# pmorenoz/HetMOGP

Measured on AMD Instinct MI355X. Metric: ELBO-steps/sec (one step = ELBO + all parameter gradients), higher is better.
Workload: dtype f64

## Files before the change

### hetmogp_amd/csrc/common.h

```cpp
#pragma once
#include <hip/hip_runtime.h>
#include <stdint.h>
#include <string>

#define HMOGP_WAVE 64
#ifndef HMOGP_POTRF_NB
#define HMOGP_POTRF_NB 32
#endif

typedef double f64x4 __attribute__((ext_vector_type(4)));
typedef double f64x2 __attribute__((ext_vector_type(2)));

struct HipError {
  hipError_t code;
  const char* what;
  const char* file;
  int line;
};
#define HIP_TRY(expr)                                          \
  do {                                                         \
    hipError_t _e = (expr);                                    \
    if (_e != hipSuccess) throw HipError{_e, #expr, __FILE__, __LINE__}; \
  } while (0)

// ... 7 lines not shown
  v = wave_sum(v);
  const int lane = threadIdx.x & 63, w = threadIdx.x >> 6, nw = (blockDim.x + 63) >> 6;
  __syncthreads();
  if (lane == 0) scratch[w] = v;
  __syncthreads();
  double r = 0.0;
  if (threadIdx.x == 0)
    for (int i = 0; i < nw; ++i) r += scratch[i];
  return r;
}

struct GemmArgs {
  const double* A = nullptr;
  const double* B = nullptr;
  double* C = nullptr;
  const double* kscale = nullptr;
  int M = 0, N = 0, K = 0;
  int lda = 0, ldb = 0, ldc = 0;
  long long sA = 0, sB = 0, sC = 0, sS = 0;
  double alpha = 1.0, beta = 0.0;
  int nbatch = 1;
  int M_last = 0, N_last = 0, K_last = 0;
  int nouter = 1;
  long long oA = 0, oB = 0, oC = 0, oS = 0;
  int ksplit = 1;
  long long sSplit = 0;
  int a_kmajor = 0, b_kmajor = 1;
  int lower_only = 0;
  int diag_balance = 1;
  int role = 0;
  double* fs_part = nullptr;
  const double* fs_a = nullptr;
  const double* fs_x = nullptr;
  const double* fs_z = nullptr;
  const double* fs_ell = nullptr;
  int fs_ldz = 0, fs_P = 1, fs_hyper = 0;
  long long fs_sPart = 0, fs_sA = 0, fs_sZ = 0;
  int store_c = 1;
  int fs_sq = 0;
  const double* fs_k = nullptr;
  const double* c_src = nullptr;
  int c_sub = 0;
  int a_tri = 0, b_tri = 0;
  const int* win = nullptr;
  long long win_stride = 0;
};
void launch_combine_parts(const double* part, int tiles, long long n, double* p, double* c, double* pt, double* ct,
                          hipStream_t s, int nb = 1, long long sPart = 0, long long ldn = 0);
void launch_gemm_f64(const GemmArgs& g, hipStream_t stream);
bool gemm_rowpass_eligible(const GemmArgs& g);
void launch_gemm_rowpass(const GemmArgs& g, hipStream_t stream);
int launch_gemm_rowpass_or_general(const GemmArgs& g, hipStream_t stream);
bool gemm_rowpass_would_take(const GemmArgs& g);
constexpr int GEMM_MAX_FWD_PARTS = 4;
bool gemm_small_eligible(const GemmArgs& g);
void launch_gemm_small(const GemmArgs& g, hipStream_t stream);

void launch_potrf_batched(double* A, int Q, int M, int* d_info, double* dscr, hipStream_t stream, int panel_begin = 0,
                          int panel_end = -1);
void launch_trtri_batched(const double* L, double* Linv, double* tmp, int Q, int M, hipStream_t stream, bool linv_is_zero = false);
void launch_ltl_batched(const double* Linv, double* Out, int Q, int M, hipStream_t stream);

void launch_fill(double* p, long long n, double v, hipStream_t stream);
void launch_unpack_tril(const double* L_flat , double* L , int Q, int M, hipStream_t s);
void launch_gemv_batched(const double* A, const double* x, double* y, int Q, int M, long long sx, int incx,
                         hipStream_t s);
```

### hetmogp_amd/csrc/engine.hip

```cpp
#include "engine_impl.h"

hipEvent_t hmogp_engine::new_event() {
  if (pool_used == pool.size()) {
    hipEvent_t e;
    HIP_TRY(hipEventCreate(&e));
    pool.push_back(e);
  }
  return pool[pool_used++];
}

void hmogp_engine::collect_spans() {
  static const bool dbg = getenv("HMOGP_DEBUG_TIMELINE") != nullptr;
  for (auto& s : spans) {
    float f = 0.f;
    if (hipEventElapsedTime(&f, s.a, s.b) == hipSuccess) ms[s.cat] += f;
    if (dbg) {
      float t0 = 0.f;
      if (hipEventElapsedTime(&t0, ev_begin0, s.a) == hipSuccess)
        std::fprintf(stderr, "[hmogp timeline] cat %d  start %9.3f ms  dur %9.3f ms\n", s.cat, t0, f);
    }
  }
  spans.clear();
  pool_used = 0;
}

hmogp_engine::~hmogp_engine() {
  drop_graphs();
  comm_destroy();
  for (auto e : pool) (void)hipEventDestroy(e);
  if (h_info2) (void)hipHostFree(h_info2);
  if (ev_ng) (void)hipEventDestroy(ev_ng);
  if (h_small) (void)hipHostFree(h_small);
  for (auto e : {ev_begin0, ev_begin1, ev_fin0, ev_fin1, ev_fork, ev_gsk, ev_zero, ev_info, ev_S, ev_join, ev_col, ev_kuf, ev_params, ev_ua, ev_qu})
    if (e) (void)hipEventDestroy(e);
  if (hstage) (void)hipHostFree(hstage);
  if (h_info) (void)hipHostFree(h_info);
  if (h_cond) (void)hipHostFree(h_cond);
  if (ev_cond) (void)hipEventDestroy(ev_cond);
  if (st2_own) (void)hipStreamDestroy(st2_own);
  if (st3_own) (void)hipStreamDestroy(st3_own);
  if (st) (void)hipStreamDestroy(st);
}

void hmogp_engine::init(const hmogp_config* c) {
  if (!c || c->abi_version != HMOGP_ABI_VERSION) throw EngineError{HMOGP_E_INVALID, "bad config / ABI version"};
  T = c->T, Q = c->Q, M = c->M, P = c->P, Df = c->Df, device = c->device;
  if (T < 1 || Q < 1 || M < 1 || Df < 1) throw EngineError{HMOGP_E_INVALID, "T, Q, M, Df must be >= 1"};
  if (P < 1 || P > 4) throw EngineError{HMOGP_E_INVALID, "input dimension P must be 1..4"};
  if (Q > HMOGP_MAXQ) throw EngineError{HMOGP_E_INVALID, "Q exceeds HMOGP_MAXQ (8)"};
  if (c->chunk_rows > 0) {
    chunk = c->chunk_rows;
  } else {
    const long long fit = (64LL << 30) / (16LL * Q * M);
    chunk = std::max<long long>(4096, std::min<long long>(1048576, fit / 1024 * 1024));
  }
  use_windows = (c->flags & HMOGP_CFG_EXACT_ZERO_WINDOWS) != 0;
  cache_kuu = (c->flags & HMOGP_CFG_CACHE_KUU) != 0;
  no_small = (c->flags & HMOGP_CFG_NO_SMALL_PATH) != 0;
  strict = strict_cfg = (c->flags & HMOGP_CFG_STRICT_QF) != 0;
  if (strict && use_windows) throw EngineError{HMOGP_E_INVALID, "HMOGP_CFG_STRICT_QF and HMOGP_CFG_EXACT_ZERO_WINDOWS exclude each other"};
  if (c->flags & ~(HMOGP_CFG_EXACT_ZERO_WINDOWS | HMOGP_CFG_CACHE_KUU | HMOGP_CFG_NO_SMALL_PATH | HMOGP_CFG_STRICT_QF))
    throw EngineError{HMOGP_E_INVALID, "unknown bits in hmogp_config.flags"};
  quirks = c->quirks;
  if (quirks & ~HMOGP_QUIRKS_REFERENCE) throw EngineError{HMOGP_E_INVALID, "unknown bits in hmogp_config.quirks"};
  if (use_windows && M > 8192) throw EngineError{HMOGP_E_INVALID, "exact-zero windows support M <= 8192"};
  int ndev = 0;
  if (hipGetDeviceCount(&ndev) != hipSuccess || ndev < 1)
    throw EngineError{HMOGP_E_NO_DEVICE, "no HIP device visible (this library has no CPU path)"};
  if (device < 0 || device >= ndev) throw EngineError{HMOGP_E_NO_DEVICE, "HIP device ordinal out of range"};
  HIP_TRY(hipSetDevice(device));
  {
    int lo = 0, hi = 0;
    HIP_TRY(hipDeviceGetStreamPriorityRange(&lo, &hi));
    HIP_TRY(hipStreamCreateWithPriority(&st, hipStreamNonBlocking, hi));
    const char* cus_env = getenv("HMOGP_ST2_CUS");
    int cus = cus_env ? atoi(cus_env) : 0;
    hipDeviceProp_t prop;
    HIP_TRY(hipGetDeviceProperties(&prop, device));
    if (cus > 0 && cus < prop.multiProcessorCount) {
      std::vector<uint32_t> mask((prop.multiProcessorCount + 31) / 32, 0u);
      for (int i = 0; i < cus; ++i) mask[i / 32] |= 1u << (i % 32);
      if (hipExtStreamCreateWithCUMask(&st2, (uint32_t)mask.size(), mask.data()) != hipSuccess) st2 = nullptr;
    }
    const char* free_env = getenv("HMOGP_ST2_FREE");
    const int nfree = free_env ? atoi(free_env) : 0;
    if (!st2 && nfree > 0 && nfree < 32 && prop.multiProcessorCount == 256) {
      const char* lay = getenv("HMOGP_ST2_LAYOUT");
      const int layout = lay ? atoi(lay) : 1;
      st2_masked = true;
      std::vector<uint32_t> mask(8, 0xFFFFFFFFu);
      for (int x = 0; x < 8; ++x)
        for (int c = 32 - nfree; c < 32; ++c) {
          const int bit = layout == 0 ? x * 32 + c : c * 8 + x;
          mask[bit / 32] &= ~(1u << (bit % 32));
        }
      if (hipExtStreamCreateWithCUMask(&st2, (uint32_t)mask.size(), mask.data()) != hipSuccess) st2 = nullptr, st2_masked = false;
    }
    if (!st2) HIP_TRY(hipStreamCreateWithPriority(&st2, hipStreamNonBlocking, lo));
    HIP_TRY(hipStreamCreateWithPriority(&st3, hipStreamNonBlocking, hi));
    st2_own = st2, st3_own = st3;
  }
  for (hipEvent_t* e : {&ev_fork, &ev_gsk, &ev_zero, &ev_info, &ev_S, &ev_join, &ev_col, &ev_kuf, &ev_params, &ev_ua, &ev_qu})
    HIP_TRY(hipEventCreateWithFlags(e, hipEventDisableTiming));
  HIP_TRY(hipEventRecord(ev_qu, st));
  HIP_TRY(hipEventRecord(ev_join, st));
  for (hipEvent_t* e : {&ev_begin0, &ev_begin1, &ev_fin0, &ev_fin1}) HIP_TRY(hipEventCreate(e));
  f_index.assign(c->f_index, c->f_index + Df);
  d_index.assign(c->d_index, c->d_index + Df);
  tasks.resize(T);
  int d = 0;
  for (int t = 0; t < T; ++t) {
    Task& k = tasks[t];
    k.lik = c->lik_id[t];
    k.param = c->lik_param ? c->lik_param[t] : 0.0;
    if (k.lik == HMOGP_LIK_GAUSSIAN && !(k.param > 0.0)) k.param = 0.5;
    k.dimf = lik_dimf(k.lik, k.param);
    check_lik_param(k.lik, k.param);
    k.qparam = k.lik == HMOGP_LIK_ORDINAL ? ordinal_table(k.param).sigma : k.param;
    if (k.dimf < 1 || k.dimf > HMOGP_MAXJ) throw EngineError{HMOGP_E_INVALID, "unsupported likelihood / dim_f"};
    k.d0 = d;
    for (int j = 0; j < k.dimf; ++j, ++d)
      if (d >= Df || f_index[d] != t || d_index[d] != j)
        throw EngineError{HMOGP_E_INVALID, "f_index / d_index inconsistent with the likelihood list"};
  }
  if (d != Df) throw EngineError{HMOGP_E_INVALID, "Df does not match the likelihood list"};
  const long long MM = (long long)M * M;
  NG = 2 + Df;
  oR = MM, oDZ = MM + M, oSA = oDZ + (long long)M * P, oSL = oSA + 1, oSWK = oSA + 2;
  per_q = oSWK + Df;
  nstats = NG + Q * per_q;
  stats.ensure(sizeof(double) * nstats, true);
  nwire = NG + Q * ((long long)M * (M + 1) / 2 + (per_q - MM));
  for (int t = 0; t < T; ++t) {
    Task& k = tasks[t];
    const int J = k.dimf;
    k.nscal = 2 + 2 * Q + J + Q * J;
    std::vector<long long> off(k.nscal);
    off[0] = 0, off[1] = 1;
    for (int q = 0; q < Q; ++q) {
      off[2 + 2 * q] = NG + q * per_q + oSA;
      off[3 + 2 * q] = NG + q * per_q + oSL;
      for (int j = 0; j < J; ++j) off[2 + 2 * Q + J + q * J + j] = NG + q * per_q + oSWK + k.d0 + j;
    }
    for (int j = 0; j < J; ++j) off[2 + 2 * Q + j] = 2 + k.d0 + j;
    k.offsets.ensure(sizeof(long long) * k.nscal);
    HIP_TRY(hipMemcpy(k.offsets.p, off.data(), sizeof(long long) * k.nscal, hipMemcpyHostToDevice));
  }
  const size_t mmq = sizeof(double) * MM * Q;
  for (DevBuf* b : {&Kuu, &Luu, &Kuui, &L, &S, &KiS, &KSK, &C, &Ctri, &Sqi, &tmpA, &tmpB, &HK, &G, &GSK, &dKmm, &dLdS}) b->ensure(mmq, true);
  oJit = 2 * Q + 2 * Q * Df, oW0 = oJit + Q, oBs = oW0 + Q * Df, oSeq = oBs + T;
  n_small = oSeq + 1;
  auto even = [](long long n) { return (n + 1) & ~1LL; };
  const long long nZ = (long long)M * Q * P, nmu = (long long)M * Q, nL = ((long long)M * (M + 1) / 2) * Q;
  oZ = even(n_small), oMu = oZ + even(nZ), oLf = oMu + even(nmu), n_params = oLf + even(nL);
  dparams.ensure(sizeof(double) * n_params);
// ... 456 lines not shown
```

### hetmogp_amd/csrc/engine_impl.h

```cpp
#pragma once
#include <algorithm>
#include <cmath>
#include <cstdio>
#include <cstdlib>
#include <cstring>
#include <string>
#include <vector>

#include <chrono>
#include <thread>

#include <dlfcn.h>
#include <hip/hip_runtime.h>
extern "C" {
typedef struct ncclComm* ncclComm_t;
}
namespace hm_nccl {
struct UniqueId { char internal[128]; };
enum : int { Success = 0, InProgress = 7, DataDouble = 8, OpSum = 0 };
using GetUniqueId = int (*)(UniqueId*);
using CommInitRank = int (*)(ncclComm_t*, int, UniqueId, int);
using CommDestroy = int (*)(ncclComm_t);
using CommAbort = int (*)(ncclComm_t);
using CommGetAsyncError = int (*)(ncclComm_t, int*);
// ... 170 lines not shown
  long long n_small = 0, oZ = 0, oMu = 0, oLf = 0, n_params = 0, oJit = 0, oW0 = 0, oBs = 0, oSeq = 0;
  int eval_seq = 0;
  DevBuf Kuu, Luu, Kuui, L, S, KiS, KSK, C, Ctri, Sqi, tmpA, tmpB, HK, G, GSK, dKmm, dLdS;
  DevBuf a, Kr, gmu, gL, klout, rowout, dinfo, djit, dscr;
  long long ws_rows = 0;
  DevBuf Kh, Pt, vp, vc, vpt, vct, valpha, vbeta, valpha0, vbeta0;
  DevBuf colred;
  DevBuf stats, wire, slabs, colpart, quadpart, fwdpart, winrow, wincol, winhit, Xws, dstage;
  long long nwire = 0;
  int* h_info = nullptr;
  double* hstage = nullptr;
  size_t hstage_cap = 0;
  bool began = false, evaluated = false;
  bool qu_resident = false;
  DevBuf ad_gms_m, ad_sms_m, ad_step_m, ad_pend_m, ad_gms_L, ad_sms_L, ad_step_L, ad_pend_L;

  struct Span {
    hipEvent_t a, b;
    int cat;
  };
  std::vector<hipEvent_t> pool;
  size_t pool_used = 0;
  std::vector<Span> spans;
  double ms[NCAT] = {0};
  long long launches[NCAT] = {0};
  hipEvent_t ev_begin0 = nullptr, ev_begin1 = nullptr, ev_fin0 = nullptr, ev_fin1 = nullptr;
  bool st2_masked = false;
  hipStream_t st2_own = nullptr, st3_own = nullptr;
  bool small_mode = false;
  bool small_path = false, small_veto = false, small_info_pending = false, info_early = false;
  double* hstage_dev = nullptr;
  bool small_rows = false;
  DevBuf smallslab;
  struct RetryRegular {};
  struct SmallGraph {
    std::vector<long long> key;
    hipGraph_t graph = nullptr;
    hipGraphExec_t exec = nullptr;
  };
  std::vector<SmallGraph> graphs;
  std::vector<std::vector<long long>> warm_keys;
  long long graph_replays = 0, graph_captures = 0;
  void drop_graphs(bool keep_warm = false);
  std::vector<long long> graph_key(const hmogp_params* p) const;
  bool graph_step(const hmogp_params* p, hmogp_outputs* out);
  bool graphs_broken = false, via_graph = false;
  std::vector<long long> pending_warm;
  void mark_warm();
  hipStream_t st2 = nullptr;
  hipStream_t st3 = nullptr;
  hipEvent_t ev_qu = nullptr;
  hipEvent_t ev_fork = nullptr, ev_gsk = nullptr, ev_zero = nullptr, ev_info = nullptr, ev_S = nullptr, ev_join = nullptr, ev_col = nullptr, ev_kuf = nullptr, ev_params = nullptr,
             ev_ua = nullptr;

  hipEvent_t new_event();
  struct Scope {
    hmogp_engine* e;
    Span s;
    hipStream_t stream;
    bool on_;
    Scope(hmogp_engine* eng, int cat, int nlaunch, hipStream_t on = nullptr) : e(eng), stream(on ? on : eng->st) {
      static const bool off = getenv("HMOGP_NO_SPANS") != nullptr;
      on_ = !off && (!eng->small_mode || cat == CAT_EXCHANGE);
      s.cat = cat;
      e->launches[cat] += nlaunch;
      if (!on_) return;
      s.a = e->new_event();
      s.b = e->new_event();
      (void)hipEventRecord(s.a, stream);
    }
    ~Scope() {
      if (!on_) return;
      (void)hipEventRecord(s.b, stream);
      e->spans.push_back(s);
    }
  };
  void collect_spans();

  ncclComm_t comm = nullptr;
  int comm_ranks = 1, comm_rank = 0;
  bool exchanged = false;

  void comm_init(int nranks, int rank, const void* id);
  void comm_destroy();
  void comm_abort();
  void wait_exchanged();
  void exchange();

  ~hmogp_engine();

  double* Hq(int q) { return stats.d() + NG + q * per_q; }

  void init(const hmogp_config* c);

  void set_task_data(int t, const double* X, const double* Y, long long N);

  void ensure_workspace(long long rows);

  long long ws_strict_rows = 0;
  void ensure_strict_workspace();

  void upload_params(const hmogp_params* p, bool enqueue = true);

  void mm(const double* A, bool a_k, const double* B, bool b_k, double* Cc, double alpha = 1.0, long long sA = -1,
          int lda = -1, hipStream_t stream = nullptr, int a_tri = 0, int b_tri = 0, bool lower_only = false) {
    GemmArgs g;
// ... 72 lines not shown
```

### hetmogp_amd/csrc/engine_rows.hip

```cpp
#include "engine_impl.h"

void hmogp_engine::u_algebra_small() {
  Scope sc(this, CAT_MM, 1);
  kuu_key_valid = false;
  if (!h_info) HIP_TRY(hipHostMalloc((void**)&h_info, sizeof(int) * HMOGP_MAXQ, hipHostMallocDefault));
  for (int q = 0; q < Q; ++q)
    if (rung[q] == -2) rung[q] = -1;
  if (!pools.empty()) {
    stage_pool_inputs(pools[0], st);
    if (!small_rows) kuf_pool(pools[0], st);
    kuf_prefetched = true;
    HIP_TRY(hipEventRecord(ev_kuf, st));
  }
  SmallU u;
  u.M = M, u.Q = Q, u.P = P, u.ldz = Q * P;
  u.Z = dZ.d(), u.var = dvar.d(), u.ell = dell.d(), u.jit = dsmall.d() + oJit, u.mu = dmu.d(), u.Lflat = dLflat.d();
  u.Kuu = Kuu.d(), u.Luu = Luu.d(), u.Kuui = Kuui.d(), u.L = L.d(), u.S = S.d(), u.KiS = KiS.d(), u.KSK = KSK.d(), u.C = C.d();
  u.Ctri = Ctri.d(), u.Sqi = Sqi.d(), u.a = a.d(), u.klout = klout.d(), u.info = dinfo.as<int>(), u.flag = dinfo.as<int>() + HMOGP_MAXQ;
  u.seq = dsmall.d() + oSeq;
  u.zero = stats.d(), u.nzero = nstats;
  launch_u_small(u, st);
  if (info_early) HIP_TRY(hipMemcpyAsync(h_info, dinfo.p, sizeof(int) * Q, hipMemcpyDeviceToHost, st));
  small_info_pending = true;
  HIP_TRY(hipEventRecord(ev_join, st));
// ... 424 lines not shown
      const bool row_sl = want_hyper && !col_sl;
      qm.p = vp.d(), qm.c = vc.d(), qm.pt = row_sl ? vpt.d() : nullptr, qm.ct = row_sl ? vct.d() : nullptr;
      qm.Wd = dW.d(), qm.W0d = dsmall.d() + oW0, qm.kapd = dkap.d(), qm.vard = dvar.d(), qm.scale_base = dsmall.d() + oBs;
      qm.quirks = quirks;
      qm.alpha = valpha.d(), qm.beta = vbeta.d(), qm.alpha0 = valpha0.d(), qm.beta0 = vbeta0.d(), qm.partials = quadpart.d();
      long long part = 0;
      for (size_t i = 0; i < pl.size(); ++i) {
        const Seg& sg = pl[i];
        Task& k = tasks[sg.t];
        QuadSeg& g = qm.seg[i];
        g.lik = k.lik, g.dimf = k.dimf, g.d0 = k.d0, g.t = sg.t, g.lik_param = k.qparam, g.N = sg.n, g.off = sg.off;
        g.y = k.quad_y() + sg.r0, g.yaux = k.Yaux.p ? k.Yaux.d() + sg.r0 : nullptr, g.ldy = k.quad_ldy();
        auto& r = qred.s[qred.nseg++];
        r.part = quadpart.d() + part, r.nrows = quad_blocks(k.lik, sg.n), r.nscal = k.nscal, r.off = k.offsets.as<long long>();
        part += r.nrows * k.nscal;
      }
      if (quad_multi || quad_multi_specialised(qm)) {
        Scope sc(this, CAT_QUAD, quad_multi ? 1 : 2);
        launch_quad_multi(qm, st);
        if (!quad_multi) launch_reduce_rows_multi(qred, stats.d(), st);
      } else {
        Scope sc(this, CAT_QUAD, 2 * (int)pl.size());
        for (auto& sg : pl) quad_segment(sg);
      }
    } else {
      Scope sc(this, CAT_QUAD, 2 * (int)pl.size());
      for (auto& sg : pl) quad_segment(sg);
    }
    if (small_rows) {
      Scope sc(this, CAT_GRAM, 2);
      launch_small_bwd(sr, st, quad_multi ? &qred : nullptr);
      continue;
    }
    colstats_rows(0, n, 0);
    {
      const int ksplit = use_windows ? std::min(8, gram_ksplit(n, M)) : gram_ksplit(n, M);
      slabs.ensure(sizeof(double) * MM * ksplit * Q, true);
      GemmArgs g;
      g.A = strict ? Ah.d() : Kh.d(), g.lda = M, g.a_kmajor = 1, g.sA = sK;
      g.B = g.A, g.ldb = M, g.b_kmajor = 1, g.sB = sK;
      g.kscale = vbeta.d(), g.sS = ldn;
      g.C = slabs.d(), g.ldc = M, g.sC = MM * ksplit;
      g.M = g.N = M, g.K = (int)n;
      g.nbatch = Q;
      g.lower_only = 1;
      g.ksplit = ksplit, g.sSplit = MM;
      g.role = 2;
      static const int bal = [] {
        const char* e = getenv("HMOGP_DIAG_BALANCE");
        return e ? atoi(e) : 1;
      }();
      g.diag_balance = bal;
      g.win = cw, g.win_stride = 2 * ncb;
      {
        Scope sc(this, CAT_GRAM, 1);
        launch_gemm_rowpass_or_general(g, st);
      }
      {
        Scope sc(this, CAT_COLSTATS, 1, st2);
        launch_reduce_slabs(colpart.d(), (int)nsp, clen, (long long)M * (1 + P), Hq(0) + oR, true, st2, Q, nsp * clen, per_q);
        if (col_sl) {
          launch_reduce_slabs(colpart.d() + (long long)M * (1 + P), (int)nsp, clen, M, colred.d(), false, st2, Q, nsp * clen, M);
          launch_sum_cols(colred.d(), Q, M, Hq(0) + oSL, per_q, st2);
        }
      }
      HIP_TRY(hipEventRecord(ev_col, st2));
      Scope sc2(this, CAT_COLSTATS, 1);
      launch_reduce_slabs_lower(slabs.d(), ksplit, M, Hq(0), true, st, Q, MM * ksplit, per_q);
    }
    HIP_TRY(hipStreamWaitEvent(st, ev_col, 0));
  }
}
```

### hetmogp_amd/csrc/gemm_rowpass.hip

```cpp
#include <cstdlib>

#include "common.h"

namespace {

constexpr int BM = 128, BN = 128, BK = 16, W = 8, NT = W * 64;
constexpr int KM_LD = 144, RM_LD = 18, TILE_DOUBLES = BK * KM_LD;
constexpr int NB = 2, WN = 32, NWN = 4;

struct Tile {
  double a[2][TILE_DOUBLES];
  double b[2][TILE_DOUBLES];
};

__device__ __forceinline__ int diag_wm(int w) { return (0x4B >> w) & 1; }
__device__ __forceinline__ int diag_wn(int w) { return (0x7E84 >> (2 * w)) & 3; }

template <int ROLE, bool FOLD = false>
__device__ __forceinline__ void rowpass_tile(const GemmArgs& g, int tiles_n, int ti, int tj, int split, Tile& lds, double* epi_a,
                                             int* hwinfo = nullptr) {
  const int batch = blockIdx.z;
  const int M = g.M, N = g.N, K = g.K;
  const int i0 = ti * BM, j0 = tj * BN;
  if (i0 >= M || j0 >= N) return;
  int wlo = 0;
  if (ROLE == 1 && g.b_tri > 0) wlo = j0;
  const int ksteps = (K - wlo + BK - 1) / BK;
  const int per = (ksteps + g.ksplit - 1) / g.ksplit;
  const int kbeg = wlo + split * per * BK;
  const int kend = min(K, kbeg + per * BK);

  const double* __restrict__ A = g.A + (long long)batch * g.sA;
  const double* __restrict__ B = g.B + (long long)batch * g.sB;
  const double* __restrict__ S = (ROLE == 2) ? g.kscale + (long long)batch * g.sS : nullptr;
  double* __restrict__ C = g.C + (long long)batch * g.sC + (long long)split * g.sSplit;
  double* fs_part = (ROLE == 1 && g.fs_part) ? g.fs_part + (long long)batch * g.fs_sPart : nullptr;

  const int t = threadIdx.x, lane = t & 63, w = __builtin_amdgcn_readfirstlane(t >> 6);
  const int lr = lane & 15, lk = lane >> 4;
  int wm = w >> 2, wn = w & 3;
  if (FOLD && w >= 4) wn = 3 - wn;
  const int klive = FOLD ? j0 + 32 * wn : 0;
  unsigned sub = 0xFFu;
  const bool diag = ROLE == 2 && ti == tj && g.lower_only;
  if (diag && hwinfo) {
    if (lane == 0) {
      const unsigned hw = __builtin_amdgcn_s_getreg(4 | (0 << 6) | (31 << 11));
      hwinfo[w] = (int)((hw >> 4) & 3u);
      if (w == 0) hwinfo[8] = (int)((hw >> 1) & 1u);
    }
  }
  constexpr bool SWAP = (ROLE == 1);
  const int blr = SWAP ? 4 * (lr & 3) + (lr >> 2) : lr;

  f64x4 acc[4][NB];
#pragma unroll
  for (int a = 0; a < 4; ++a)
#pragma unroll
    for (int b = 0; b < NB; ++b) acc[a][b] = f64x4{0.0, 0.0, 0.0, 0.0};

  const int ar = t >> 2, ak = (t & 3) * 4, bk = t >> 5, bc = (t & 31) * 2;
  const double* pa;
  const double* pb;
  if (ROLE == 1) {
    pa = A + (long long)min(i0 + ar, M - 1) * g.lda + ak;
    pb = B + (long long)bk * g.ldb + j0 + bc;
  } else {
    pa = A + i0 + bc;
    pb = B + j0 + bc;
  }
  double ra[4], rb[4], ks = 1.0;
  auto load = [&](int k0) {
    if (ROLE == 1) {
      const f64x2 x0 = *reinterpret_cast<const f64x2*>(pa + k0), x1 = *reinterpret_cast<const f64x2*>(pa + k0 + 2);
      ra[0] = x0.x, ra[1] = x0.y, ra[2] = x1.x, ra[3] = x1.y;
      const double* q = pb + (long long)k0 * g.ldb;
      const f64x2 y0 = *reinterpret_cast<const f64x2*>(q), y1 = *reinterpret_cast<const f64x2*>(q + 64);
      rb[0] = y0.x, rb[1] = y0.y, rb[2] = y1.x, rb[3] = y1.y;
    } else {
      const int row = k0 + bk;
      const long long off = (long long)min(row, K - 1) * g.lda;
      const f64x2 x0 = *reinterpret_cast<const f64x2*>(pa + off), x1 = *reinterpret_cast<const f64x2*>(pa + off + 64);
      ra[0] = x0.x, ra[1] = x0.y, ra[2] = x1.x, ra[3] = x1.y;
      const f64x2 y0 = *reinterpret_cast<const f64x2*>(pb + off), y1 = *reinterpret_cast<const f64x2*>(pb + off + 64);
      rb[0] = y0.x, rb[1] = y0.y, rb[2] = y1.x, rb[3] = y1.y;
      ks = (row < kend) ? S[row] : 0.0;
    }
  };
  auto stage = [&](int buf) {
    if (ROLE == 1) {
      double* sa = &lds.a[buf][ar * RM_LD + ak];
      *reinterpret_cast<f64x2*>(sa) = f64x2{ra[0], ra[1]};
      *reinterpret_cast<f64x2*>(sa + 2) = f64x2{ra[2], ra[3]};
    } else {
      double* sa = &lds.a[buf][bk * KM_LD + bc];
      *reinterpret_cast<f64x2*>(sa) = f64x2{ra[0], ra[1]};
      *reinterpret_cast<f64x2*>(sa + 64) = f64x2{ra[2], ra[3]};
#pragma unroll
      for (int i = 0; i < 4; ++i) rb[i] *= ks;
    }
    double* sb = &lds.b[buf][bk * KM_LD + bc];
    *reinterpret_cast<f64x2*>(sb) = f64x2{rb[0], rb[1]};
    *reinterpret_cast<f64x2*>(sb + 64) = f64x2{rb[2], rb[3]};
  };
  double fa[2][4], fb[2][NB];
  auto frag = [&](int buf, int kk, int s) {
    const double* fpa = (ROLE == 1) ? &lds.a[buf][(wm * 64 + lr) * RM_LD + kk * 4 + lk] : &lds.a[buf][(kk * 4 + lk) * KM_LD + wm * 64 + lr];
    const double* fpb = &lds.b[buf][(kk * 4 + lk) * KM_LD + wn * WN + blr];
#pragma unroll
    for (int i = 0; i < 4; ++i) fa[s][i] = fpa[i * 16 * (ROLE == 1 ? RM_LD : 1)];
#pragma unroll
    for (int i = 0; i < NB; ++i) fb[s][i] = fpb[i * 16];
  };
  auto mm8 = [&](int s) {
#pragma unroll
    for (int a = 0; a < 4; ++a)
#pragma unroll
      for (int b = 0; b < NB; ++b) {
        if (ROLE == 2 && !((sub >> (a * NB + b)) & 1u)) continue;
        acc[a][b] = SWAP ? __builtin_amdgcn_mfma_f64_16x16x4f64(fb[s][b], fa[s][a], acc[a][b], 0, 0, 0)
                         : __builtin_amdgcn_mfma_f64_16x16x4f64(fa[s][a], fb[s][b], acc[a][b], 0, 0, 0);
      }
  };

  int cur = 0;
  if (kbeg < kend) {
    load(kbeg);
    stage(0);
    if (kbeg + BK < kend) load(kbeg + BK);
  }
  __syncthreads();
  if (diag) {
    int role = w;
    if (hwinfo) {
      bool ok = true;
      unsigned seen = 0;
#pragma unroll
      for (int i = 0; i < 4; ++i) {
        ok = ok && hwinfo[i] == hwinfo[i + 4];
        seen |= 1u << hwinfo[i];
      }
      if (ok && seen == 0xFu) role = ((hwinfo[w] + 2 * hwinfo[8]) & 3) + (w & 4);
    }
    role = __builtin_amdgcn_readfirstlane(role);
    wm = diag_wm(role), wn = diag_wn(role);
    sub = 0;
#pragma unroll
    for (int a = 0; a < 4; ++a)
#pragma unroll
      for (int b = 0; b < NB; ++b)
        if (wn * NB + b <= wm * 4 + a) sub |= 1u << (a * NB + b);
  }
  const bool live = ROLE == 1 || sub != 0;
  if (ROLE == 2) {
    for (int k0 = kbeg; k0 < kend; k0 += BK) {
      if (k0 + BK < kend) stage(cur ^ 1);
      if (k0 + 2 * BK < kend) load(k0 + 2 * BK);
      if (live) {
#pragma unroll
        for (int kk = 0; kk < BK / 4; ++kk) {
          frag(cur, kk, 0);
          mm8(0);
        }
      }
      __syncthreads();
      cur ^= 1;
    }
  }
  if (ROLE == 1 && kbeg < kend && (!FOLD || kbeg >= klive)) frag(0, 0, 0);
#define HM_SB __builtin_amdgcn_sched_barrier(0)
  for (int k0 = kbeg; ROLE == 1 && k0 < kend; k0 += BK) {
    const bool more = k0 + BK < kend;
    const bool lv = !FOLD || k0 >= klive;
    if (lv) {
      frag(cur, 1, 1);
      HM_SB;
      mm8(0);
      HM_SB;
    }
    if (more) stage(cur ^ 1);
    if (k0 + 2 * BK < kend) load(k0 + 2 * BK);
    HM_SB;
    if (lv) {
      frag(cur, 2, 0);
      HM_SB;
      mm8(1);
      HM_SB;
      frag(cur, 3, 1);
      HM_SB;
      mm8(0);
      HM_SB;
    }
    __syncthreads();
    if (more && (!FOLD || k0 + BK >= klive)) frag(cur ^ 1, 0, 0);
    if (lv) {
      HM_SB;
      mm8(1);
      HM_SB;
    }
    cur ^= 1;
  }
#undef HM_SB

  if (ROLE == 1 && fs_part && g.fs_sq) {
#pragma unroll
    for (int a = 0; a < 4; ++a) {
// ... 46 lines not shown
        for (int r = 0; r < 4; ++r) {
          sp += kv[r] * av[r];
          sc += acc[a][b][r] * kv[r];
        }
      }
#pragma unroll
      for (int o = 16; o <= 32; o <<= 1) {
        sp += __shfl_xor(sp, o, 64);
        sc += __shfl_xor(sc, o, 64);
      }
      if (lk == 0 && i0 + rl < M) {
        double* o = fs_part + ((long long)(NWN * tj + wn)) * M + (i0 + rl);
        const long long ss = (long long)NWN * tiles_n * M;
        o[0] = sp, o[ss] = sc;
      }
      if (a < 2) {
        asm volatile("" ::: "memory");
        issue(a + 2);
      }
    }
    if (!g.store_c) return;
  }
  if (SWAP) {
#pragma unroll
    for (int a = 0; a < 4; ++a) {
      const int row = i0 + wm * 64 + a * 16 + lr;
      if (row >= M) continue;
      double* crow = C + (long long)row * g.ldc + j0 + wn * WN + 4 * lk;
      if (g.c_sub) {
        const double* srow = g.c_src ? g.c_src + (long long)batch * g.sC + (long long)row * g.ldc + j0 + wn * WN + 4 * lk : crow;
#pragma unroll
        for (int b = 0; b < NB; ++b) {
          const f64x2 c01 = *reinterpret_cast<const f64x2*>(srow + b * 16), c23 = *reinterpret_cast<const f64x2*>(srow + b * 16 + 2);
          *reinterpret_cast<f64x2*>(crow + b * 16) = f64x2{c01.x - acc[a][b][0], c01.y - acc[a][b][1]};
          *reinterpret_cast<f64x2*>(crow + b * 16 + 2) = f64x2{c23.x - acc[a][b][2], c23.y - acc[a][b][3]};
        }
        continue;
      }
#pragma unroll
      for (int b = 0; b < NB; ++b) {
        *reinterpret_cast<f64x2*>(crow + b * 16) = f64x2{acc[a][b][0], acc[a][b][1]};
        *reinterpret_cast<f64x2*>(crow + b * 16 + 2) = f64x2{acc[a][b][2], acc[a][b][3]};
      }
    }
    return;
  }
#pragma unroll
  for (int a = 0; a < 4; ++a)
#pragma unroll
    for (int r = 0; r < 4; ++r) {
      double* crow = C + (long long)(i0 + wm * 64 + a * 16 + 4 * r + lk) * g.ldc + j0 + wn * WN + lr;
#pragma unroll
      for (int b = 0; b < NB; ++b)
        if ((sub >> (a * NB + b)) & 1u) crow[b * 16] = acc[a][b][r];
    }
}

template <int ROLE, bool PAIR>
__device__ __forceinline__ void rowpass_block(const GemmArgs& g, int tiles_n, int ntiles, Tile& lds, double* epi_a,
                                              int* hwinfo = nullptr) {

  int v = blockIdx.x, split = 0;
  int ti, tj;
  if (ROLE == 2 && g.lower_only) {
    const int T = tiles_n, noff = T * (T - 1) / 2, ks8 = (g.ksplit > 1) ? ((g.ksplit + 7) / 8) * 8 : 1, gx1 = noff * ks8;
    if (v < gx1) {
      int u = v;
      if (g.ksplit > 1) {
        const int xcd = v & 7, idx = v >> 3;
        split = (idx / noff) * 8 + xcd;
        u = idx % noff;
      }
      ti = (int)((sqrt(8.0 * (double)u + 1.0) + 1.0) * 0.5);
      while (ti * (ti + 1) / 2 <= u) ++ti;
      while (ti * (ti - 1) / 2 > u) --ti;
      tj = u - ti * (ti - 1) / 2;
    } else {
      const int u = v - gx1;
      split = u / T;
      ti = tj = u - split * T;
    }
    if (split >= g.ksplit) return;
  } else {
    if (g.ksplit > 1) {
      const int xcd = v & 7, idx = v >> 3;
      split = (idx / ntiles) * 8 + xcd;
      v = idx % ntiles;
      if (split >= g.ksplit) return;
    } else if ((ntiles & 7) == 0) {
      const int cpx = ntiles >> 3;
      v = (v & 7) * cpx + (v >> 3);
    }
    const int tcols = PAIR ? tiles_n / 2 : tiles_n;
    ti = v / tcols;
    tj = v - ti * tcols;
  }
  rowpass_tile<ROLE, PAIR>(g, tiles_n, ti, tj, split, lds, epi_a, hwinfo);
  if (PAIR) {
    __syncthreads();
    rowpass_tile<ROLE, PAIR>(g, tiles_n, ti, tiles_n - 1 - tj, split, lds, epi_a);
  }
}

template <int ROLE>
__global__ __launch_bounds__(NT, 4) void rowpass_gemm_kernel(GemmArgs g, int tiles_n, int ntiles) {
  __shared__ __attribute__((aligned(16))) Tile lds;
  __shared__ __attribute__((aligned(16))) double epi_a[ROLE == 1 ? 128 : 2];
  __shared__ int hwinfo[ROLE == 2 ? 16 : 1];
  rowpass_block<ROLE, false>(g, tiles_n, ntiles, lds, epi_a, (ROLE == 2 && g.diag_balance) ? hwinfo : nullptr);
}
__global__ __launch_bounds__(NT, 4) void rowpass_fold_pair_kernel(GemmArgs g, int tiles_n, int ntiles) {
  __shared__ __attribute__((aligned(16))) Tile lds;
  __shared__ __attribute__((aligned(16))) double epi_a[128];
  rowpass_block<1, true>(g, tiles_n, ntiles, lds, epi_a);
}

bool aligned16(const void* p) { return (((uintptr_t)p) & 15) == 0; }

}

bool gemm_rowpass_eligible(const GemmArgs& g) {
  const bool sub = g.role == 1 && g.alpha == -1.0 && g.beta == 1.0 && !g.fs_part && g.b_tri == 0 && g.store_c;
  if (g.nouter != 1 || (!sub && (g.alpha != 1.0 || g.beta != 0.0)) || g.win || g.M_last || g.N_last || g.K_last || g.a_tri) return false;
  if ((g.lda & 1) || (g.ldb & 1) || (g.ldc & 1) || !aligned16(g.A) || !aligned16(g.B) || !aligned16(g.C)) return false;
  if (g.c_src && (!sub || !aligned16(g.c_src))) return false;
  if (g.fs_k && (g.role != 1 || !g.fs_part || g.fs_sq || !aligned16(g.fs_k))) return false;
  if ((g.sA & 1) || (g.sB & 1) || (g.sC & 1) || (g.sSplit & 1)) return false;
  if (g.role == 1)
    return !g.a_kmajor && g.b_kmajor && !g.lower_only && g.ksplit == 1 && !g.kscale && g.b_tri >= 0 && (g.N % BN) == 0 &&
           (g.K % BK) == 0 && (g.K == g.N || sub) && g.K >= BK && g.M >= 1;
  if (g.role == 2)
    return g.a_kmajor && g.b_kmajor && g.kscale && g.b_tri == 0 && g.M == g.N && (g.N % BN) == 0 &&
           g.lda == g.ldb && g.K >= 1;
  return false;
}

void launch_gemm_rowpass(const GemmArgs& g_in, hipStream_t stream) {
  GemmArgs g = g_in;
  g.c_sub = (g.role == 1 && g.alpha == -1.0 && g.beta == 1.0) ? 1 : 0;
  const int tiles_m = (g.M + BM - 1) / BM, tiles_n = (g.N + BN - 1) / BN;
  const int ntiles = g.lower_only ? tiles_m * (tiles_m + 1) / 2 : tiles_m * tiles_n;
  const int gx = (g.ksplit > 1) ? ntiles * ((g.ksplit + 7) / 8) * 8 : ntiles;
  dim3 grid(gx, 1, g.nbatch);
  if (g.role == 1) {
    const int pair = (g.b_tri > 0 && g.ksplit == 1 && tiles_n >= 2 && (tiles_n & 1) == 0) ? 1 : 0;
    if (pair) {
      grid.x = tiles_m * (tiles_n / 2);
      hipLaunchKernelGGL(rowpass_fold_pair_kernel, grid, dim3(NT), 0, stream, g, tiles_n, (int)grid.x);
    } else {
      hipLaunchKernelGGL((rowpass_gemm_kernel<1>), grid, dim3(NT), 0, stream, g, tiles_n, ntiles);
    }
  } else {
    hipLaunchKernelGGL((rowpass_gemm_kernel<2>), grid, dim3(NT), 0, stream, g, tiles_n, ntiles);
  }
}

static bool rowpass_enabled() {
  static const bool enabled = [] {
    const char* e = getenv("HMOGP_ROWPASS");
    return !(e && e[0] == '0');
  }();
  return enabled;
}
bool gemm_rowpass_would_take(const GemmArgs& g) { return rowpass_enabled() && gemm_rowpass_eligible(g); }

int launch_gemm_rowpass_or_general(const GemmArgs& g, hipStream_t stream) {
  const bool enabled = rowpass_enabled();
  if ((g.fs_sq || g.fs_k) && !(enabled && gemm_rowpass_eligible(g)))
    throw HipError{hipErrorInvalidValue, "fs_sq / fs_k are features of the specialised forward kernel only", __FILE__, __LINE__};
  if (enabled && gemm_rowpass_eligible(g)) {
    launch_gemm_rowpass(g, stream);
    return NWN;
  }
  if (g.role == 1 && (g.alpha != 1.0 || g.beta != 0.0)) {
    GemmArgs h = g;
    h.role = 0;
    launch_gemm_f64(h, stream);
    return 2;
  }
  launch_gemm_f64(g, stream);
  return 2;
}
```

Before: 8.379.

## Split gram rowpass into off-diagonal and dedicated diagonal kernels on separate streams

Adds a Gram path that separates the lower-triangular off-diagonal tiles from the diagonal tiles. Off-diagonal tiles use the general tile code with the per-subtile triangle guard compiled out. Diagonal tiles get a specialised kernel where each wave computes only its share of lower-triangle 16x16 subtiles. By default (HMOGP_GRAM_SPLIT=1) the diagonal kernel runs on the high-priority stream st3, joined back with events, so the two kernels can overlap. This aims to remove divergent wasted work and load imbalance on diagonal tiles, at the cost of an extra launch and event synchronisation.

```diff
diff --git a/hetmogp_amd/csrc/common.h b/hetmogp_amd/csrc/common.h
--- a/hetmogp_amd/csrc/common.h
+++ b/hetmogp_amd/csrc/common.h
@@ -83,6 +83,9 @@
 void launch_gemm_rowpass(const GemmArgs& g, hipStream_t stream);
 int launch_gemm_rowpass_or_general(const GemmArgs& g, hipStream_t stream);
 bool gemm_rowpass_would_take(const GemmArgs& g);
+void launch_gram_rowpass_lower(const GemmArgs& g, hipStream_t stream);
+void launch_gram_rowpass_diag(const GemmArgs& g, hipStream_t stream);
+void launch_gram_rowpass_phases(const GemmArgs& g, hipStream_t stream);
 constexpr int GEMM_MAX_FWD_PARTS = 4;
 bool gemm_small_eligible(const GemmArgs& g);
 void launch_gemm_small(const GemmArgs& g, hipStream_t stream);
diff --git a/hetmogp_amd/csrc/engine.hip b/hetmogp_amd/csrc/engine.hip
--- a/hetmogp_amd/csrc/engine.hip
+++ b/hetmogp_amd/csrc/engine.hip
@@ -31,7 +31,7 @@
   if (h_info2) (void)hipHostFree(h_info2);
   if (ev_ng) (void)hipEventDestroy(ev_ng);
   if (h_small) (void)hipHostFree(h_small);
-  for (auto e : {ev_begin0, ev_begin1, ev_fin0, ev_fin1, ev_fork, ev_gsk, ev_zero, ev_info, ev_S, ev_join, ev_col, ev_kuf, ev_params, ev_ua, ev_qu})
+  for (auto e : {ev_begin0, ev_begin1, ev_fin0, ev_fin1, ev_fork, ev_gsk, ev_zero, ev_info, ev_S, ev_join, ev_col, ev_kuf, ev_params, ev_ua, ev_qu, ev_gfork, ev_gjoin})
     if (e) (void)hipEventDestroy(e);
   if (hstage) (void)hipHostFree(hstage);
   if (h_info) (void)hipHostFree(h_info);
@@ -100,7 +100,7 @@
     HIP_TRY(hipStreamCreateWithPriority(&st3, hipStreamNonBlocking, hi));
     st2_own = st2, st3_own = st3;
   }
-  for (hipEvent_t* e : {&ev_fork, &ev_gsk, &ev_zero, &ev_info, &ev_S, &ev_join, &ev_col, &ev_kuf, &ev_params, &ev_ua, &ev_qu})
+  for (hipEvent_t* e : {&ev_fork, &ev_gsk, &ev_zero, &ev_info, &ev_S, &ev_join, &ev_col, &ev_kuf, &ev_params, &ev_ua, &ev_qu, &ev_gfork, &ev_gjoin})
     HIP_TRY(hipEventCreateWithFlags(e, hipEventDisableTiming));
   HIP_TRY(hipEventRecord(ev_qu, st));
   HIP_TRY(hipEventRecord(ev_join, st));
diff --git a/hetmogp_amd/csrc/engine_impl.h b/hetmogp_amd/csrc/engine_impl.h
--- a/hetmogp_amd/csrc/engine_impl.h
+++ b/hetmogp_amd/csrc/engine_impl.h
@@ -246,6 +246,7 @@
   hipEvent_t ev_qu = nullptr;
   hipEvent_t ev_fork = nullptr, ev_gsk = nullptr, ev_zero = nullptr, ev_info = nullptr, ev_S = nullptr, ev_join = nullptr, ev_col = nullptr, ev_kuf = nullptr, ev_params = nullptr,
              ev_ua = nullptr;
+  hipEvent_t ev_gfork = nullptr, ev_gjoin = nullptr;
 
   hipEvent_t new_event();
   struct Scope {
diff --git a/hetmogp_amd/csrc/engine_rows.hip b/hetmogp_amd/csrc/engine_rows.hip
--- a/hetmogp_amd/csrc/engine_rows.hip
+++ b/hetmogp_amd/csrc/engine_rows.hip
@@ -500,7 +500,27 @@
       }();
       g.diag_balance = bal;
       g.win = cw, g.win_stride = 2 * ncb;
-      {
+      static const int gram_split = [] {
+        const char* e = getenv("HMOGP_GRAM_SPLIT");
+        return e ? atoi(e) : 1;
+      }();
+      if (gram_split == 4 && gemm_rowpass_would_take(g)) {
+        Scope sc(this, CAT_GRAM, 1);
+        launch_gram_rowpass_phases(g, st);
+      } else if (gram_split >= 1 && gram_split <= 3 && gemm_rowpass_would_take(g)) {
+        Scope sc(this, CAT_GRAM, M > 128 ? 2 : 1);
+        hipStream_t sd = gram_split == 1 ? st3 : gram_split == 2 ? st2 : st;
+        if (sd != st) {
+          HIP_TRY(hipEventRecord(ev_gfork, st));
+          HIP_TRY(hipStreamWaitEvent(sd, ev_gfork, 0));
+        }
+        launch_gram_rowpass_lower(g, st);
+        launch_gram_rowpass_diag(g, sd);
+        if (sd != st) {
+          HIP_TRY(hipEventRecord(ev_gjoin, sd));
+          HIP_TRY(hipStreamWaitEvent(st, ev_gjoin, 0));
+        }
+      } else {
         Scope sc(this, CAT_GRAM, 1);
         launch_gemm_rowpass_or_general(g, st);
       }
diff --git a/hetmogp_amd/csrc/gemm_rowpass.hip b/hetmogp_amd/csrc/gemm_rowpass.hip
--- a/hetmogp_amd/csrc/gemm_rowpass.hip
+++ b/hetmogp_amd/csrc/gemm_rowpass.hip
@@ -16,7 +16,7 @@
 __device__ __forceinline__ int diag_wm(int w) { return (0x4B >> w) & 1; }
 __device__ __forceinline__ int diag_wn(int w) { return (0x7E84 >> (2 * w)) & 3; }
 
-template <int ROLE, bool FOLD = false>
+template <int ROLE, bool FOLD = false, bool NODIAG = false>
 __device__ __forceinline__ void rowpass_tile(const GemmArgs& g, int tiles_n, int ti, int tj, int split, Tile& lds, double* epi_a,
                                              int* hwinfo = nullptr) {
   const int batch = blockIdx.z;
@@ -42,7 +42,8 @@
   if (FOLD && w >= 4) wn = 3 - wn;
   const int klive = FOLD ? j0 + 32 * wn : 0;
   unsigned sub = 0xFFu;
-  const bool diag = ROLE == 2 && ti == tj && g.lower_only;
+  constexpr bool GUARD = ROLE == 2 && !NODIAG;
+  const bool diag = GUARD && ti == tj && g.lower_only;
   if (diag && hwinfo) {
     if (lane == 0) {
       const unsigned hw = __builtin_amdgcn_s_getreg(4 | (0 << 6) | (31 << 11));
@@ -117,7 +118,7 @@
     for (int a = 0; a < 4; ++a)
 #pragma unroll
       for (int b = 0; b < NB; ++b) {
-        if (ROLE == 2 && !((sub >> (a * NB + b)) & 1u)) continue;
+        if (GUARD && !((sub >> (a * NB + b)) & 1u)) continue;
         acc[a][b] = SWAP ? __builtin_amdgcn_mfma_f64_16x16x4f64(fb[s][b], fa[s][a], acc[a][b], 0, 0, 0)
                          : __builtin_amdgcn_mfma_f64_16x16x4f64(fa[s][a], fb[s][b], acc[a][b], 0, 0, 0);
       }
@@ -151,7 +152,7 @@
       for (int b = 0; b < NB; ++b)
         if (wn * NB + b <= wm * 4 + a) sub |= 1u << (a * NB + b);
   }
-  const bool live = ROLE == 1 || sub != 0;
+  const bool live = !GUARD || sub != 0;
   if (ROLE == 2) {
     for (int k0 = kbeg; k0 < kend; k0 += BK) {
       if (k0 + BK < kend) stage(cur ^ 1);
@@ -304,8 +305,22 @@
       double* crow = C + (long long)(i0 + wm * 64 + a * 16 + 4 * r + lk) * g.ldc + j0 + wn * WN + lr;
 #pragma unroll
       for (int b = 0; b < NB; ++b)
-        if ((sub >> (a * NB + b)) & 1u) crow[b * 16] = acc[a][b][r];
-    }
+        if (!GUARD || ((sub >> (a * NB + b)) & 1u)) crow[b * 16] = acc[a][b][r];
+    }
+}
+
+__device__ __forceinline__ void gram_lower_decode(int v, int noff, int ksplit, int& ti, int& tj, int& split) {
+  int u = v;
+  split = 0;
+  if (ksplit > 1) {
+    const int xcd = v & 7, idx = v >> 3;
+    split = (idx / noff) * 8 + xcd;
+    u = idx % noff;
+  }
+  ti = (int)((sqrt(8.0 * (double)u + 1.0) + 1.0) * 0.5);
+  while (ti * (ti + 1) / 2 <= u) ++ti;
+  while (ti * (ti - 1) / 2 > u) --ti;
+  tj = u - ti * (ti - 1) / 2;
 }
 
 template <int ROLE, bool PAIR>
@@ -317,16 +332,7 @@
   if (ROLE == 2 && g.lower_only) {
     const int T = tiles_n, noff = T * (T - 1) / 2, ks8 = (g.ksplit > 1) ? ((g.ksplit + 7) / 8) * 8 : 1, gx1 = noff * ks8;
     if (v < gx1) {
-      int u = v;
-      if (g.ksplit > 1) {
-        const int xcd = v & 7, idx = v >> 3;
-        split = (idx / noff) * 8 + xcd;
-        u = idx % noff;
-      }
-      ti = (int)((sqrt(8.0 * (double)u + 1.0) + 1.0) * 0.5);
-      while (ti * (ti + 1) / 2 <= u) ++ti;
-      while (ti * (ti - 1) / 2 > u) --ti;
-      tj = u - ti * (ti - 1) / 2;
+      gram_lower_decode(v, noff, g.ksplit, ti, tj, split);
     } else {
       const int u = v - gx1;
       split = u / T;
@@ -365,6 +371,146 @@
   __shared__ __attribute__((aligned(16))) Tile lds;
   __shared__ __attribute__((aligned(16))) double epi_a[128];
   rowpass_block<1, true>(g, tiles_n, ntiles, lds, epi_a);
+}
+
+
+__global__ __launch_bounds__(NT, 4) void rowpass_gram_lower_kernel(GemmArgs g, int tiles_n) {
+  __shared__ __attribute__((aligned(16))) Tile lds;
+  __shared__ __attribute__((aligned(16))) double epi_a[2];
+  int ti, tj, split;
+  gram_lower_decode(blockIdx.x, tiles_n * (tiles_n - 1) / 2, g.ksplit, ti, tj, split);
+  if (split >= g.ksplit) return;
+  rowpass_tile<2, false, true>(g, tiles_n, ti, tj, split, lds, epi_a);
+}
+
+__device__ __forceinline__ unsigned diag_slots(int w) {
+  switch (w) {
+    case 0: return 0u | 1u << 3 | 6u << 6 | 0u << 9 | 1u << 12 | 0u << 15 | 1u << 18;
+    case 1: return 2u | 3u << 3 | 4u << 6 | 2u << 9 | 3u << 12 | 2u << 15 | 3u << 18;
+    case 2: return 4u | 5u << 3 | 5u << 6 | 4u << 9 | 5u << 12 | 2u << 15 | 3u << 18;
+    case 3: return 6u | 7u << 3 | 7u << 6 | 6u << 9 | 7u << 12 | 0u << 15 | 1u << 18;
+    case 4: return 2u | 3u << 3 | 2u << 6 | 0u << 9 | 1u << 12 | 0u << 15 | 1u << 18;
+    case 5: return 4u | 5u << 3 | 4u << 6 | 0u << 9 | 1u << 12 | 0u << 15 | 1u << 18;
+    case 6: return 6u | 7u << 3 | 6u << 6 | 2u << 9 | 3u << 12 | 2u << 15 | 3u << 18;
+    default: return 6u | 7u << 3 | 6u << 6 | 4u << 9 | 5u << 12 | 4u << 15 | 5u << 18;
+  }
+}
+
+template <bool FIVE>
+__device__ __forceinline__ void gram_diag_tile(const GemmArgs& g, int d, int split, int w, Tile& lds) {
+  const int batch = blockIdx.z;
+  const int K = g.K, i0 = d * BM;
+  const int ksteps = (K + BK - 1) / BK;
+  const int per = (ksteps + g.ksplit - 1) / g.ksplit;
+  const int kbeg = split * per * BK;
+  const int kend = min(K, kbeg + per * BK);
+
+  const double* __restrict__ A = g.A + (long long)batch * g.sA;
+  const double* __restrict__ S = g.kscale + (long long)batch * g.sS;
+  double* __restrict__ C = g.C + (long long)batch * g.sC + (long long)split * g.sSplit;
+
+  const int t = threadIdx.x, lane = t & 63;
+  const int lr = lane & 15, lk = lane >> 4;
+  const unsigned slots = diag_slots(w);
+  int sa[3], sb[4];
+#pragma unroll
+  for (int i = 0; i < 3; ++i) sa[i] = (int)((slots >> (3 * i)) & 7u);
+#pragma unroll
+  for (int i = 0; i < 4; ++i) sb[i] = (int)((slots >> (9 + 3 * i)) & 7u);
+  constexpr int NS = FIVE ? 5 : 4;
+  f64x4 acc[NS];
+#pragma unroll
+  for (int i = 0; i < NS; ++i) acc[i] = f64x4{0.0, 0.0, 0.0, 0.0};
+
+  const int bk = t >> 5, bc = (t & 31) * 2;
+  const double* pa = A + i0 + bc;
+  double ra[4], ks = 1.0;
+  auto load = [&](int k0) {
+    const int row = k0 + bk;
+    const long long off = (long long)min(row, K - 1) * g.lda;
+    const f64x2 x0 = *reinterpret_cast<const f64x2*>(pa + off), x1 = *reinterpret_cast<const f64x2*>(pa + off + 64);
+    ra[0] = x0.x, ra[1] = x0.y, ra[2] = x1.x, ra[3] = x1.y;
+    ks = (row < kend) ? S[row] : 0.0;
+  };
+  auto stage = [&](int buf) {
+    double* pa_ = &lds.a[buf][bk * KM_LD + bc];
+    *reinterpret_cast<f64x2*>(pa_) = f64x2{ra[0], ra[1]};
+    *reinterpret_cast<f64x2*>(pa_ + 64) = f64x2{ra[2], ra[3]};
+    double* pb_ = &lds.b[buf][bk * KM_LD + bc];
+    *reinterpret_cast<f64x2*>(pb_) = f64x2{ra[0] * ks, ra[1] * ks};
+    *reinterpret_cast<f64x2*>(pb_ + 64) = f64x2{ra[2] * ks, ra[3] * ks};
+  };
+  auto step = [&](int buf, int kk) {
+    const double* fpa = &lds.a[buf][(kk * 4 + lk) * KM_LD + lr];
+    const double* fpb = &lds.b[buf][(kk * 4 + lk) * KM_LD + lr];
+    const double a0 = fpa[sa[0] * 16], a1 = fpa[sa[1] * 16];
+    const double b0 = fpb[sb[0] * 16], b1 = fpb[sb[1] * 16];
+    acc[0] = __builtin_amdgcn_mfma_f64_16x16x4f64(a0, b0, acc[0], 0, 0, 0);
+    acc[1] = __builtin_amdgcn_mfma_f64_16x16x4f64(a1, b0, acc[1], 0, 0, 0);
+    acc[2] = __builtin_amdgcn_mfma_f64_16x16x4f64(a1, b1, acc[2], 0, 0, 0);
+    if (FIVE) {
+      const double a2 = fpa[sa[2] * 16], b2 = fpb[sb[2] * 16], b3 = fpb[sb[3] * 16];
+      acc[3] = __builtin_amdgcn_mfma_f64_16x16x4f64(a2, b2, acc[3], 0, 0, 0);
+      acc[NS - 1] = __builtin_amdgcn_mfma_f64_16x16x4f64(a2, b3, acc[NS - 1], 0, 0, 0);
+    } else {
+      acc[3] = __builtin_amdgcn_mfma_f64_16x16x4f64(a0, b1, acc[3], 0, 0, 0);
+    }
+  };
+
+  int cur = 0;
+  if (kbeg < kend) {
+    load(kbeg);
+    stage(0);
+    if (kbeg + BK < kend) load(kbeg + BK);
+  }
+  __syncthreads();
+  for (int k0 = kbeg; k0 < kend; k0 += BK) {
+    if (k0 + BK < kend) stage(cur ^ 1);
+    if (k0 + 2 * BK < kend) load(k0 + 2 * BK);
+#pragma unroll
+    for (int kk = 0; kk < BK / 4; ++kk) step(cur, kk);
+    __syncthreads();
+    cur ^= 1;
+  }
+
+  auto store = [&](int i, int a, int b) {
+#pragma unroll
+    for (int r = 0; r < 4; ++r) C[(long long)(i0 + a * 16 + 4 * r + lk) * g.ldc + i0 + b * 16 + lr] = acc[i][r];
+  };
+  store(0, sa[0], sb[0]);
+  store(1, sa[1], sb[0]);
+  store(2, sa[1], sb[1]);
+  if (FIVE) {
+    store(3, sa[2], sb[2]);
+    store(NS - 1, sa[2], sb[3]);
+  } else {
+    store(3, sa[0], sb[1]);
+  }
+}
+
+__global__ __launch_bounds__(NT, 4) void rowpass_gram_diag_kernel(GemmArgs g, int tiles_n) {
+  __shared__ __attribute__((aligned(16))) Tile lds;
+  const int v = blockIdx.x, split = v / tiles_n, d = v - split * tiles_n;
+  if (split >= g.ksplit) return;
+  const int w = __builtin_amdgcn_readfirstlane(threadIdx.x >> 6);
+  if (w < 4) gram_diag_tile<true>(g, d, split, w, lds);
+  else gram_diag_tile<false>(g, d, split, w, lds);
+}
+__global__ __launch_bounds__(NT, 4) void rowpass_gram_phases_kernel(GemmArgs g, int tiles_n) {
+  __shared__ __attribute__((aligned(16))) Tile lds;
+  const int noff = tiles_n * (tiles_n - 1) / 2, ks8 = (g.ksplit > 1) ? ((g.ksplit + 7) / 8) * 8 : 1, gx1 = noff * ks8;
+  if ((int)blockIdx.x < gx1) {
+    int ti, tj, split;
+    gram_lower_decode(blockIdx.x, noff, g.ksplit, ti, tj, split);
+    if (split >= g.ksplit) return;
+    rowpass_tile<2, false, true>(g, tiles_n, ti, tj, split, lds, nullptr);
+    return;
+  }
+  const int v = blockIdx.x - gx1, split = v / tiles_n, d = v - split * tiles_n;
+  if (split >= g.ksplit) return;
+  const int w = __builtin_amdgcn_readfirstlane(threadIdx.x >> 6);
+  if (w < 4) gram_diag_tile<true>(g, d, split, w, lds);
+  else gram_diag_tile<false>(g, d, split, w, lds);
 }
 
 bool aligned16(const void* p) { return (((uintptr_t)p) & 15) == 0; }
@@ -407,6 +553,22 @@
   }
 }
 
+void launch_gram_rowpass_lower(const GemmArgs& g, hipStream_t stream) {
+  const int T = (g.N + BN - 1) / BN, noff = T * (T - 1) / 2;
+  if (noff == 0) return;
+  const int ks8 = (g.ksplit > 1) ? ((g.ksplit + 7) / 8) * 8 : 1;
+  hipLaunchKernelGGL(rowpass_gram_lower_kernel, dim3(noff * ks8, 1, g.nbatch), dim3(NT), 0, stream, g, T);
+}
+void launch_gram_rowpass_phases(const GemmArgs& g, hipStream_t stream) {
+  const int T = (g.N + BN - 1) / BN, noff = T * (T - 1) / 2;
+  const int ks8 = (g.ksplit > 1) ? ((g.ksplit + 7) / 8) * 8 : 1;
+  hipLaunchKernelGGL(rowpass_gram_phases_kernel, dim3(noff * ks8 + T * g.ksplit, 1, g.nbatch), dim3(NT), 0, stream, g, T);
+}
+void launch_gram_rowpass_diag(const GemmArgs& g, hipStream_t stream) {
+  const int T = (g.N + BN - 1) / BN;
+  hipLaunchKernelGGL(rowpass_gram_diag_kernel, dim3(T * g.ksplit, 1, g.nbatch), dim3(NT), 0, stream, g, T);
+}
+
 static bool rowpass_enabled() {
   static const bool enabled = [] {
     const char* e = getenv("HMOGP_ROWPASS");
```

New measurement: 8.402, median of 6. No clear change (+0.3%).
